# cvsp-lab/ICLR2025_3D-MOM

Hardware: AMD Instinct MI355X
Metric: 4DGS train-steps/sec @200k Gaussians, 960×540, 60 frames; render FPS (higher is better)
Workload: dtype f32; 1 GPU; 200k Gaussians, 60 frames, 960x540, HexPlane on; gaussians=200000, frames=60, width=960, height=540, parallelism=single, ranks_seen=1, gaussians_at_end=200000, steps_replayed_after_overflow=0

## Files before the change

### iclr2025_3d-mom_amd/_native.py

```python
from __future__ import annotations

import ctypes as C
import os
import subprocess

_HERE = os.path.dirname(os.path.abspath(__file__))
LIB_PATH = os.environ.get("MOM4D_LIB") or os.path.join(_HERE, "lib", "libmom4d.so")
_lib = None

MOM_OK, MOM_EINVAL, MOM_ELAUNCH, MOM_ECAPACITY, MOM_EUNAVAILABLE = 0, -1, -2, -3, -4
_ERR = {MOM_EINVAL: "invalid argument", MOM_ELAUNCH: "HIP launch/runtime failure", MOM_ECAPACITY: "scratch too small",
        MOM_EUNAVAILABLE: "run-time dependency missing (librccl)"}
COMM_F32, COMM_I32, COMM_SUM, COMM_MAX = 0, 1, 0, 1


class MomError(RuntimeError):
    pass


GACC_FLOATS = int(os.environ.get("MOM_GACC_FLOATS", "12"))
ABI_VERSION = 8


class MomRasterArgs(C.Structure):
    _fields_ = [("struct_size", C.c_uint),
                ("P", C.c_int), ("D", C.c_int), ("M", C.c_int), ("W", C.c_int), ("H", C.c_int),
                ("background", C.c_void_p), ("means3D", C.c_void_p), ("shs", C.c_void_p), ("shs_rest", C.c_void_p),
                ("colors_precomp", C.c_void_p), ("opacities", C.c_void_p), ("scales", C.c_void_p),
                ("rotations", C.c_void_p), ("cov3D_precomp", C.c_void_p), ("viewmatrix", C.c_void_p),
                ("projmatrix", C.c_void_p), ("campos", C.c_void_p), ("scale_modifier", C.c_float),
                ("tan_fovx", C.c_float), ("tan_fovy", C.c_float), ("prefiltered", C.c_int), ("debug", C.c_int),
                ("tile_row0", C.c_int), ("tile_row1", C.c_int),
                ("forward_only", C.c_int),
                ("overflow_tag", C.c_uint),
                ("keep_all_tiles", C.c_int),
                ("l1_target", C.c_void_p), ("l1_grad", C.c_void_p), ("l1_sums", C.c_void_p),
                ("accum_cleared", C.c_int),
                ("l1_partials", C.c_void_p),
                ("status_post", C.c_void_p), ("status_serial", C.c_uint),
                ("l1_grad_scale", C.c_float),
                ("params_raw", C.c_int)]

    def __init__(self, *args, **kw):
        super().__init__(*args, **kw)
        self.struct_size = C.sizeof(type(self))


class MomRasterGrads(C.Structure):
    _fields_ = [(n, C.c_void_p) for n in ("dL_dmeans2D", "dL_dcolors", "dL_dopacity", "dL_dmeans3D", "dL_dcov3D",
                                          "dL_dsh", "dL_dsh_rest", "dL_dscales", "dL_drotations", "act_rotations_raw",
                                          "dL_dscales_copy", "dL_drotations_copy",
                                          "stats_max_radii2D", "stats_grad_accum", "stats_denom", "stats_skip_if_nonzero")]


class MomRasterAccum(C.Structure):
    _fields_ = [("struct_size", C.c_uint),
                ("dL_dmeans3D_copy", C.c_void_p),
                ("radii_max", C.c_void_p)]

    def __init__(self, *args, **kw):
# ... 283 lines not shown
```

### iclr2025_3d-mom_amd/csrc/raster_api.hip

```cpp
#include "mom_common.h"

int mom_launch_preprocess_fwd(const MomRasterArgs* a, const GeomView& g, int* radii, uint32_t* zero_words, int n_zero, hipStream_t s);
int mom_launch_mark_visible(int P, const float* means3D, const float* view, uint8_t* present, hipStream_t s);
int mom_launch_binning_count(const MomRasterArgs* a, const GeomView& g, const ImageView& im, uint32_t* num_rendered_dev,
                             uint32_t* num_rendered_host, hipStream_t s);
int mom_launch_binning_sort(const MomRasterArgs* a, const GeomView& g, const BinView& b, const ImageView& im, size_t capacity,
                            uint32_t* status_dev, bool render_sorts_small, hipStream_t s);
int mom_launch_render_fwd(const MomRasterArgs* a, const GeomView& g, const BinView& b, const ImageView& im, size_t capacity,
                          float* out_color, float* out_depth, bool sort_small, hipStream_t s);
int mom_launch_render_bwd(const MomRasterArgs* a, const GeomView& g, const BinView& b, const ImageView& im, size_t capacity,
                          const float* dL_dpix, const float* dL_ddepth, hipStream_t s);
int mom_launch_preprocess_bwd(const MomRasterArgs* a, const int* radii, const GeomView& g, const MomRasterGrads* gr, const MomRasterAccum* acc,
                              hipStream_t s);

static int check_args(const MomRasterArgs* a)
{
    if (!a || a->struct_size != sizeof(MomRasterArgs)) return MOM_EINVAL;
    if (a->P < 0 || a->W <= 0 || a->H <= 0) return MOM_EINVAL;
    if (a->tile_row0 < 0 || a->tile_row1 < a->tile_row0 || a->tile_row1 > (a->H + MOM_TILE - 1) / MOM_TILE) return MOM_EINVAL;
    if (a->params_raw && (a->cov3D_precomp || !a->scales || !a->rotations)) return MOM_EINVAL;
    if (a->P == 0) return MOM_OK;
    if (!a->means3D || !a->opacities || !a->viewmatrix || !a->projmatrix || !a->campos || !a->background) return MOM_EINVAL;
    if (!a->shs && !a->colors_precomp) return MOM_EINVAL;
    if (!a->cov3D_precomp && (!a->scales || !a->rotations)) return MOM_EINVAL;
    if (a->shs && !a->colors_precomp && (a->D < 0 || a->D > 3 || a->M < (a->D + 1) * (a->D + 1))) return MOM_EINVAL;
    return MOM_OK;
// ... 70 lines not shown
    out->bin_keys = (size_t)((char*)b.keys - z);
    out->bin_point_list = (size_t)((char*)b.point_list - z);
    out->img_tile_counts = (size_t)((char*)im.tile_counts - z);
    out->img_tile_walked = (size_t)((char*)im.tile_cursor - z);
    return MOM_OK;
}

int mom_raster_forward_geometry(const MomRasterArgs* a, void* geom, void* image, int* radii,
                                uint32_t* num_rendered_dev, uint32_t* num_rendered_host, mom_stream_t stream)
{
    int rc = check_args(a);
    if (rc) return rc;
    hipStream_t s = (hipStream_t)stream;
    if (!num_rendered_dev) return MOM_EINVAL;
    if (a->P == 0) {
        if (hipMemsetAsync(num_rendered_dev, 0, 4, s) != hipSuccess) return MOM_ELAUNCH;
        if (num_rendered_host) *num_rendered_host = 0;
        return MOM_OK;
    }
    if (!geom || !image || !radii) return MOM_EINVAL;
    GeomView g; ImageView im;
    geom_view(mom_align_ptr(geom), a->P, &g);
    image_view(mom_align_ptr(image), a->W, a->H, &im);
    const int tiles = ((a->W + MOM_TILE - 1) / MOM_TILE) * ((a->H + MOM_TILE - 1) / MOM_TILE);
    rc = mom_launch_preprocess_fwd(a, g, radii, im.hdr, (int)((im.tile_counts + tiles) - im.hdr), s);
    if (rc) return rc;
    MOM_CHECK_LAUNCH(a, s);
    rc = mom_launch_binning_count(a, g, im, num_rendered_dev, num_rendered_host, s);
    if (rc) return rc;
    MOM_CHECK_LAUNCH(a, s);
    return MOM_OK;
}

int mom_raster_forward_render(const MomRasterArgs* a, void* geom, void* binning, size_t capacity, void* image,
                              float* out_color, float* out_depth, uint32_t* status_dev, mom_stream_t stream)
{
    int rc = check_args(a);
    if (rc) return rc;
    hipStream_t s = (hipStream_t)stream;
    if (!out_color || !out_depth) return MOM_EINVAL;
    const size_t HW = (size_t)a->W * a->H;
    if (a->P == 0) {
        if (hipMemsetAsync(out_color, 0, HW * 12, s) != hipSuccess) return MOM_ELAUNCH;
        if (hipMemsetAsync(out_depth, 0, HW * 4, s) != hipSuccess) return MOM_ELAUNCH;
        return MOM_OK;
    }
    if (!geom || !binning || !image) return MOM_EINVAL;
    GeomView g; ImageView im; BinView b;
// ... 111 lines not shown
```

### iclr2025_3d-mom_amd/csrc/raster_bin_dev.h

```cpp
#pragma once
#include "mom_common.h"

namespace {

#ifndef MOM_SMALL_RECT
#define MOM_SMALL_RECT 24
#endif
constexpr int kSmallRect = MOM_SMALL_RECT;
constexpr int kMaxLdsTiles = 16384;


struct Reach {
    float cx, cy, a, b, c, bound, inv_a, inv_c;
    int cull;
};
__device__ __forceinline__ bool tile_reached(const Reach& r, int tx, int ty)
{
    if (!r.cull) return true;
    const float xa = (float)(tx * MOM_TILE), ya = (float)(ty * MOM_TILE);
    return mom_rect_reach(r.cx, r.cy, r.a, r.b, r.c, r.bound, r.inv_a, r.inv_c, xa, xa + (float)(MOM_TILE - 1), ya,
                          ya + (float)(MOM_TILE - 1));
}
__device__ __forceinline__ float bcast(float v, int src) { return __int_as_float(__builtin_amdgcn_readlane(__float_as_int(v), src)); }

// ... 42 lines not shown
    while (big) {
        const int src = __ffsll((long long)big) - 1;
        big &= big - 1;
        const WaveSplat b = bcast_splat(x0, y0, w, cnt, 0u, 0ull, rc, src);
        const float inv_w = __builtin_amdgcn_rcpf((float)b.w);
        for (int base = 0; base < b.cnt; base += MOM_WAVE) {
            const int i = base + lane;
            bool r = false;
            if (i < b.cnt) {
                const int q = small_div(i, inv_w);
                const int tx = b.x0 + i - q * b.w, ty = b.y0 + q;
                r = tile_reached(b.rc, tx, ty);
                if (r) f(ty * gx + tx);
            }
            if (base == 0) {
                const uint64_t bal = __ballot(r);
                if (lane == src) mask = bal;
            }
        }
    }
    return mask;
}


}

template <bool LOCAL_STAGES, class KeyPtr>
__device__ __forceinline__ void bitonic_sort(KeyPtr k, int n, int nthreads, int tid)
{
    int lm = 0;
    while ((1 << lm) < n) lm++;
    if (lm == 0) return;
    if (lm == 1) {
        __syncthreads();
        if (tid == 0) { const uint64_t ka = k[0], kb = k[1]; if (ka > kb) { k[0] = kb; k[1] = ka; } }
        __syncthreads();
        return;
    }
    const int quarter_m = (1 << lm) >> 2;
    constexpr uint64_t kInf = ~0ull;
    bool prev_wide = true;
    auto sync_before = [&](int span) {
        const bool wide = !LOCAL_STAGES || span > 256;
        if (wide || prev_wide) __syncthreads();
        else __builtin_amdgcn_wave_barrier();
        prev_wide = wide;
// ... 34 lines not shown
                cx(k0, k1); cx(k2, k3);
                st4(i0, i1, i2, i3, k0, k1, k2, k3);
            }
        }
        int lj = lk - 3;
        for (; lj >= 1; lj -= 2) {
            const int j = 1 << lj, h = j >> 1;
            sync_before(2 * j);
            for (int g = tid; g < quarter_m; g += nthreads) {
                const int x = ((g >> (lj - 1)) << (lj + 1)) | (g & (h - 1));
                const int i0 = x, i1 = x + h, i2 = x + j, i3 = x + j + h;
                if (i1 < n) {
                    uint64_t k0 = k[i0], k1 = k[i1], k2 = ld(i2), k3 = ld(i3);
                    cx(k0, k2); cx(k1, k3);
                    cx(k0, k1); cx(k2, k3);
                    st4(i0, i1, i2, i3, k0, k1, k2, k3);
                }
            }
        }
        if (lj == 0) pairs_pass();
    }
    __syncthreads();
}


constexpr int kRenderSortCap = 1536;
```

### iclr2025_3d-mom_amd/csrc/raster_binning.hip

```cpp
#include "raster_bin_dev.h"

namespace {

constexpr int kSortLdsCap = 8192;
#ifndef MOM_SORT_SMALL
#define MOM_SORT_SMALL 2048
#endif
constexpr int kSortSmallCap = MOM_SORT_SMALL;
constexpr int kOrderBins = 128;

template <class F>
__device__ __forceinline__ void for_each_kept(int x0, int y0, int x1, int y1, int gx, uint32_t payload, uint64_t mask, const Reach& rc, F f)
{
    const int lane = mom_lane();
    const int w = x1 - x0;
    const int cnt = w * (y1 - y0);
    const bool own = cnt <= MOM_WAVE && __popcll(mask) <= kSmallRect;
    if (own && cnt > 0) {
        const float inv_w = __builtin_amdgcn_rcpf((float)w);
        uint64_t m = mask;
        while (m) {
            const int i = __ffsll((long long)m) - 1;
            m &= m - 1;
            const int q = small_div(i, inv_w);
            f((y0 + q) * gx + x0 + i - q * w, lane, payload);
        }
    }
    unsigned long long big = __ballot(!own && cnt > 0);
    while (big) {
        const int src = __ffsll((long long)big) - 1;
        big &= big - 1;
        const WaveSplat b = bcast_splat(x0, y0, w, cnt, payload, mask, rc, src);
        const float inv_w = __builtin_amdgcn_rcpf((float)b.w);
        for (int base = 0; base < b.cnt; base += MOM_WAVE) {
            const int i = base + lane;
            if (i < b.cnt) {
                const int q = small_div(i, inv_w);
                const int tx = b.x0 + i - q * b.w, ty = b.y0 + q;
                const bool r = base == 0 ? ((b.mask >> lane) & 1) : tile_reached(b.rc, tx, ty);
                if (r) f(ty * gx + tx, src, b.payload);
            }
        }
    }
}

struct RectIn {
    float4 r0, r1;
    int radius;
};
__device__ __forceinline__ RectIn fetch_rect(const float4* __restrict__ rec, int g, int P)
{
    RectIn in;
    in.r0 = in.r1 = make_float4(0.f, 0.f, 0.f, 0.f);
    in.radius = 0;
    if (g < P) {
        in.r0 = rec[3 * (size_t)g];
        in.r1 = rec[3 * (size_t)g + 1];
        in.radius = __float_as_int(rec[3 * (size_t)g + 2].w);
    }
    return in;
}
__device__ __forceinline__ void make_rect(const RectIn& in, int gx, int gy, int ry0, int ry1, int cull,
                                          int& x0, int& y0, int& x1, int& y1, uint32_t& depth_bits, Reach& rc)
{
    x0 = y0 = x1 = y1 = 0;
    depth_bits = 0;
    rc = Reach{0.f, 0.f, 0.f, 0.f, 0.f, 0.f, 0.f, 0.f, 0};
    const float4 r0 = in.r0, r1 = in.r1;
    const int radius = in.radius;
    asm volatile("" :: "v"(r0.x), "v"(r0.y), "v"(r0.z), "v"(r1.x), "v"(r1.y), "v"(r1.z), "v"(r1.w), "v"(radius));
    if (radius > 0) {
        mom_get_rect(r0.x, r0.y, radius, gx, gy, x0, y0, x1, y1);
        y0 = max(y0, ry0);
        y1 = min(y1, ry1);
        if (y1 <= y0) x0 = y0 = x1 = y1 = 0;
        depth_bits = __float_as_uint(r0.z);
        if (cull && r1.x > 0.f && r1.z > 0.f)
            rc = Reach{r0.x, r0.y, r1.x, r1.y, r1.z, mom_power_bound(r1.w), __builtin_amdgcn_rcpf(r1.x), __builtin_amdgcn_rcpf(r1.z), 1};
    }
}

template <bool LDS_HIST>
__global__ void __launch_bounds__(256) tile_hist_kernel(int P, int chunks, int gx, int gy, int ry0, int ry1, int cull, const float4* __restrict__ rec,
                                                       uint32_t* __restrict__ tile_counts, unsigned long long* __restrict__ reach)
{
    extern __shared__ uint32_t s_cnt[];
    const int tiles = gx * gy;
    if (LDS_HIST) {
        for (int t = threadIdx.x; t < tiles; t += 256) s_cnt[t] = 0;
        __syncthreads();
    }
    for (int c = 0; c < chunks; c++) {
        const int g = (blockIdx.x * chunks + c) * 256 + threadIdx.x;
        int x0, y0, x1, y1;
        uint32_t db;
        Reach rc;
        make_rect(fetch_rect(rec, g, P), gx, gy, ry0, ry1, cull, x0, y0, x1, y1, db, rc);
        const uint64_t mask = decide_instances(x0, y0, x1, y1, gx, rc, [&](int tile) {
            if (LDS_HIST)
                atomicAdd(&s_cnt[tile], 1u);
            else
                atomicAdd(&tile_counts[tile], 1u);
        });
        if (g < P) reach[g] = mask;
    }
    if (LDS_HIST) {
        __syncthreads();
        for (int t = threadIdx.x; t < tiles; t += 256) {
            const uint32_t n = s_cnt[t];
            if (n) atomicAdd(&tile_counts[t], n);
        }
    }
}

__global__ void __launch_bounds__(1024) tile_scan_kernel(int tiles, const uint32_t* __restrict__ tile_counts,
                                                        uint32_t* __restrict__ tile_cursor, uint2* __restrict__ ranges,
                                                        uint32_t* __restrict__ hdr, uint32_t* __restrict__ num_rendered_dev,
                                                        uint32_t* __restrict__ num_rendered_host, int t0, int nt,
                                                        uint32_t* __restrict__ tile_order)
{
    __shared__ uint32_t s_wave[16];
    __shared__ uint32_t s_carry;
    __shared__ uint32_t s_bin[kOrderBins + 1];
    __shared__ uint32_t s_big;
    const int lane = threadIdx.x & 63, wave = threadIdx.x >> 6;
    if (threadIdx.x == 0) s_carry = 0;
    for (int i = threadIdx.x; i <= kOrderBins; i += 1024) s_bin[i] = 0;
    auto bin_of = [&](uint32_t n) { return kOrderBins - 1 - (int)min((uint32_t)(kOrderBins - 1), n >> 5); };
    __syncthreads();
    for (int base = 0; base < tiles; base += 1024) {
        const int t = base + threadIdx.x;
        const uint32_t n = t < tiles ? tile_counts[t] : 0u;
        if (t >= t0 && t < t0 + nt) atomicAdd(&s_bin[bin_of(n) + 1], 1u);
        uint32_t incl = n;
#pragma unroll
        for (int d = 1; d < 64; d <<= 1) {
            const uint32_t o = __shfl_up(incl, d);
            if (lane >= d) incl += o;
        }
        if (lane == 63) s_wave[wave] = incl;
        __syncthreads();
        uint32_t woff = 0;
        for (int w = 0; w < wave; w++) woff += s_wave[w];
        const uint32_t carry = s_carry;
        const uint32_t start = carry + woff + incl - n;
        if (t < tiles) {
            tile_cursor[t] = start;
            ranges[t] = n ? make_uint2(start, start + n) : make_uint2(0u, 0u);
        }
        __syncthreads();
        if (threadIdx.x == 1023) s_carry = start + n;
        __syncthreads();
    }
    if (threadIdx.x < 64) {
        static_assert(kOrderBins == 128, "two classes per lane of one wave");
        const uint32_t c0 = s_bin[2 * lane + 1], c1 = s_bin[2 * lane + 2];
        uint32_t incl = c0 + c1;
#pragma unroll
        for (int d = 1; d < 64; d <<= 1) {
            const uint32_t o = __shfl_up(incl, d);
            if (lane >= d) incl += o;
        }
        const uint32_t excl = incl - (c0 + c1);
        s_bin[2 * lane] = excl;
        s_bin[2 * lane + 1] = excl + c0;
        static_assert(kRenderSortCap % 32 == 0 && kRenderSortCap / 32 < kOrderBins, "class boundary");
        constexpr int kFirstSmall = kOrderBins - kRenderSortCap / 32;
        if (2 * lane == kFirstSmall) s_big = excl;
        if (2 * lane + 1 == kFirstSmall) s_big = excl + c0;
    }
    __syncthreads();
    for (int t = t0 + threadIdx.x; t < t0 + nt; t += 1024) tile_order[atomicAdd(&s_bin[bin_of(tile_counts[t])], 1u)] = (uint32_t)t;
    if (threadIdx.x == 0) {
        hdr[0] = s_carry;
        hdr[3] = (uint32_t)t0;
        hdr[4] = (uint32_t)nt;
        hdr[5] = s_big;
        *num_rendered_dev = s_carry;
        if (num_rendered_host) __hip_atomic_store(num_rendered_host, s_carry, __ATOMIC_RELAXED, __HIP_MEMORY_SCOPE_SYSTEM);
    }
}

template <bool LDS_HIST>
__global__ void __launch_bounds__(256) tile_scatter_kernel(int P, int chunks, int gx, int gy, int ry0, int ry1, int cull, const float4* __restrict__ rec,
                                                          const unsigned long long* __restrict__ reach,
                                                          uint32_t* __restrict__ tile_cursor, uint64_t* __restrict__ keys,
                                                          uint32_t capacity, uint32_t* __restrict__ hdr, uint32_t* __restrict__ sticky,
                                                          uint32_t tag)
{
    extern __shared__ uint32_t s_cnt[];
    const int tiles = gx * gy;
    bool overflow = false;
    const int g_first = blockIdx.x * chunks * 256 + threadIdx.x;
    RectIn in = fetch_rect(rec, g_first, P);
    unsigned long long rmask = g_first < P ? reach[g_first] : 0ull;
    int x0 = 0, y0 = 0, x1 = 0, y1 = 0;
    uint32_t db = 0;
    Reach rc;
    if (LDS_HIST) {
        for (int t = threadIdx.x; t < tiles; t += 256) s_cnt[t] = 0;
        __syncthreads();
        for (int c = 0; c < chunks; c++) {
            const int g = (blockIdx.x * chunks + c) * 256 + threadIdx.x;
            if (c) {
                rmask = g < P ? reach[g] : 0ull;
                in = fetch_rect(rec, g, P);
            }
            make_rect(in, gx, gy, ry0, ry1, cull, x0, y0, x1, y1, db, rc);
            for_each_kept(x0, y0, x1, y1, gx, 0u, rmask, rc, [&](int tile, int, uint32_t) { atomicAdd(&s_cnt[tile], 1u); });
        }
        __syncthreads();
        for (int t0 = threadIdx.x; t0 < tiles; t0 += 8 * 256) {
            uint32_t n[8], base[8];
#pragma unroll
            for (int k = 0; k < 8; k++) n[k] = t0 + 256 * k < tiles ? s_cnt[t0 + 256 * k] : 0u;
#pragma unroll
            for (int k = 0; k < 8; k++) base[k] = n[k] ? atomicAdd(&tile_cursor[t0 + 256 * k], n[k]) : 0u;
#pragma unroll
            for (int k = 0; k < 8; k++)
                if (n[k]) s_cnt[t0 + 256 * k] = base[k];
        }
        __syncthreads();
    }
    for (int c = 0; c < chunks; c++) {
        const int g = (blockIdx.x * chunks + c) * 256 + threadIdx.x;
        const int wave_g0 = g - mom_lane();
        if (chunks > 1 || !LDS_HIST) {
            rmask = g < P ? reach[g] : 0ull;
            if (c || LDS_HIST) in = fetch_rect(rec, g, P);
            make_rect(in, gx, gy, ry0, ry1, cull, x0, y0, x1, y1, db, rc);
        }
        for_each_kept(x0, y0, x1, y1, gx, db, rmask, rc, [&](int tile, int src, uint32_t sdb) {
            const uint32_t pos = LDS_HIST ? atomicAdd(&s_cnt[tile], 1u) : atomicAdd(&tile_cursor[tile], 1u);
            if (pos < capacity)
                keys[pos] = ((uint64_t)sdb << 32) | (uint32_t)(wave_g0 + src);
            else
                overflow = true;
        });
    }
    if (overflow) {
        atomicOr(&hdr[1], 1u);
        if (sticky) atomicCAS(sticky, 0u, tag);
    }
}

template <int LO, int CAP>
__global__ void __launch_bounds__(256) tile_sort_kernel(const uint2* __restrict__ ranges, const uint32_t* __restrict__ tile_order,
                                                       uint64_t* __restrict__ keys, uint32_t* __restrict__ point_list, uint32_t capacity,
                                                       const uint32_t* __restrict__ head_count, int nt)
{
    __shared__ uint64_t s_keys[CAP];
    const int limit = head_count ? min((int)*head_count, nt) : nt;
    for (int slot = blockIdx.x; slot < limit; slot += gridDim.x) {
        const uint2 r = ranges[tile_order[slot]];
        uint32_t end = r.y < capacity ? r.y : capacity;
        if (r.x >= end) continue;
        const int n = (int)(end - r.x);
        if (n <= LO || (n > CAP && CAP < kSortLdsCap)) continue;
        uint64_t* gk = keys + r.x;
        __syncthreads();
        if (n <= CAP) {
            for (int i = threadIdx.x; i < n; i += 256) s_keys[i] = gk[i];
            __syncthreads();
            if (n > 1) bitonic_sort<true>(s_keys, n, 256, threadIdx.x);
            for (int i = threadIdx.x; i < n; i += 256) point_list[r.x + i] = (uint32_t)s_keys[i];
        } else {
            __syncthreads();
            bitonic_sort<false>(gk, n, 256, threadIdx.x);
            __threadfence_block();
            for (int i = threadIdx.x; i < n; i += 256) point_list[r.x + i] = (uint32_t)gk[i];
        }
    }
}

}

static int bin_chunks(int P)
{
    const int chunks = (P + 256 * 2048 - 1) / (256 * 2048);
    return chunks < 1 ? 1 : chunks;
}

int mom_launch_binning_count(const MomRasterArgs* a, const GeomView& g, const ImageView& im, uint32_t* num_rendered_dev,
                             uint32_t* num_rendered_host, hipStream_t s)
{
    const int gx = (a->W + MOM_TILE - 1) / MOM_TILE, gy = (a->H + MOM_TILE - 1) / MOM_TILE;
    const int tiles = gx * gy;
    int ry0, ry1;
    mom_tile_rows(a, gy, &ry0, &ry1);
    const int cull = a->keep_all_tiles ? 0 : 1;
    const int chunks = bin_chunks(a->P);
    const int blocks = (a->P + 256 * chunks - 1) / (256 * chunks);
    mom_prof_begin(MOM_P_HIST, s);
    if (tiles <= kMaxLdsTiles)
        hipLaunchKernelGGL(tile_hist_kernel<true>, dim3(blocks), dim3(256), (size_t)tiles * 4, s, a->P, chunks, gx, gy, ry0, ry1, cull,
                           g.rec, im.tile_counts, g.reach);
    else
        hipLaunchKernelGGL(tile_hist_kernel<false>, dim3(blocks), dim3(256), 0, s, a->P, chunks, gx, gy, ry0, ry1, cull, g.rec,
                           im.tile_counts, g.reach);
    mom_prof_end(MOM_P_HIST, s);
    if (hipGetLastError() != hipSuccess) return MOM_ELAUNCH;
    MomProfScope ps(MOM_P_SCAN, s);
    hipLaunchKernelGGL(tile_scan_kernel, dim3(1), dim3(1024), 0, s, tiles, im.tile_counts, im.tile_cursor, im.ranges, im.hdr,
                       num_rendered_dev, num_rendered_host, gx * ry0, gx * (ry1 - ry0), im.tile_order);
    return hipGetLastError() == hipSuccess ? MOM_OK : MOM_ELAUNCH;
}

int mom_launch_binning_sort(const MomRasterArgs* a, const GeomView& g, const BinView& b, const ImageView& im, size_t capacity,
                            uint32_t* status_dev, bool render_sorts_small, hipStream_t s)
{
    const int gx = (a->W + MOM_TILE - 1) / MOM_TILE, gy = (a->H + MOM_TILE - 1) / MOM_TILE;
    const int tiles = gx * gy;
    int ry0, ry1;
    mom_tile_rows(a, gy, &ry0, &ry1);
    const int cull = a->keep_all_tiles ? 0 : 1;
    const int chunks = bin_chunks(a->P);
    const int blocks = (a->P + 256 * chunks - 1) / (256 * chunks);
    const uint32_t cap = capacity > 0xFFFFFFFFull ? 0xFFFFFFFFu : (uint32_t)capacity;
    const uint32_t tag = a->overflow_tag ? a->overflow_tag : 1u;
    mom_prof_begin(MOM_P_SCATTER, s);
    if (tiles <= kMaxLdsTiles)
        hipLaunchKernelGGL(tile_scatter_kernel<true>, dim3(blocks), dim3(256), (size_t)tiles * 4, s, a->P, chunks, gx, gy,
                           ry0, ry1, cull, g.rec, g.reach, im.tile_cursor, b.keys, cap, im.hdr, status_dev, tag);
    else
        hipLaunchKernelGGL(tile_scatter_kernel<false>, dim3(blocks), dim3(256), 0, s, a->P, chunks, gx, gy, ry0, ry1, cull, g.rec,
                           g.reach, im.tile_cursor, b.keys, cap, im.hdr, status_dev, tag);
    mom_prof_end(MOM_P_SCATTER, s);
    if (hipGetLastError() != hipSuccess) return MOM_ELAUNCH;
    MomProfScope ps(MOM_P_SORT, s);
    const int nt = gx * (ry1 - ry0);
    if (nt == 0) return MOM_OK;
    if (render_sorts_small) {
        hipLaunchKernelGGL((tile_sort_kernel<kRenderSortCap, kSortLdsCap>), dim3(nt < 128 ? nt : 128), dim3(256), 0, s, im.ranges,
                           im.tile_order, b.keys, b.point_list, cap, im.hdr + 5, nt);
        return hipGetLastError() == hipSuccess ? MOM_OK : MOM_ELAUNCH;
    }
    hipLaunchKernelGGL((tile_sort_kernel<0, kSortSmallCap>), dim3(nt), dim3(256), 0, s, im.ranges, im.tile_order, b.keys, b.point_list,
                       cap, (const uint32_t*)nullptr, nt);
    if (hipGetLastError() != hipSuccess) return MOM_ELAUNCH;
    hipLaunchKernelGGL((tile_sort_kernel<kSortSmallCap, kSortLdsCap>), dim3(nt), dim3(256), 0, s, im.ranges, im.tile_order, b.keys,
                       b.point_list, cap, (const uint32_t*)nullptr, nt);
    return hipGetLastError() == hipSuccess ? MOM_OK : MOM_ELAUNCH;
}
```

### iclr2025_3d-mom_amd/fused_render.py

```python
import ctypes as C
from collections import deque

import torch

from . import _native as N
from . import ops
from .diff_gaussian_rasterization import _C as RC


class FusedRender:
    def __init__(self, gaussians):
        self.g = gaussians
        self.lib = N.lib()
        self.key = None
        self.cap = 0
        self.binning = None
        self._desc_key = None
        self.serial = 0
        self.pending = deque()
        self.collect = False
        self.bad = []

    def _ensure(self, P, W, H, dev):
        if self.key == (P, W, H, dev):
# ... 93 lines not shown

    def _raster(self, a, P, W, H, dev, s):
        lib = self.lib
        a.forward_only = 1
        color = torch.empty((3, H, W), dtype=torch.float32, device=dev)
        depth = torch.empty((1, H, W), dtype=torch.float32, device=dev)
        radii = torch.empty(P, dtype=torch.int32, device=dev)
        prev_R = int(self.nr_host[0])
        late = self.overflowed(self.FLAG_LAG) if len(self.pending) > self.FLAG_LAG else []
        if late and self.collect:
            self.bad += late
        elif late:
            raise N.MomError(f"async render(): frames {late} overflowed the binning capacity and are incomplete; render them "
                             "again (the capacity has been raised), collect such frames with FusedRender.overflowed(), or use "
                             "set_sync_mode('exact')")
        wait_for_count = RC._state["mode"] == "exact" or self.cap == 0
        if wait_for_count:
            if getattr(self, "_unwaited", False):
                torch.cuda.current_stream(dev).synchronize()
                self._unwaited = False
            self.nr_host[0] = RC.COUNT_PENDING
        else:
            self._unwaited = True
        N.check(lib.mom_raster_forward_geometry(C.byref(a), self.geom.data_ptr(), self.img.data_ptr(), radii.data_ptr(),
                                                self.nr_dev.data_ptr(), self.nr_host.data_ptr(), s), "raster_geometry")
        if wait_for_count:
            count = RC.wait_count(self.nr_host)
            want = count + (0 if RC._state["mode"] == "exact" else count // 2 + 65536)
        else:
            want = max(self.cap, int(prev_R * self.HEADROOM) + self.MARGIN, getattr(self, "cap_floor", 0))
        if self.binning is None or want > self.cap or want < self.cap // 4:
            self.cap = want
            self.binning = torch.empty(lib.mom_raster_binning_bytes(P, W, H, self.cap), dtype=torch.uint8, device=dev)
        self.serial += 1
        post = RC._state["mode"] != "exact"
        if post:
            slot = self.serial % self.RING
            a.status_post, a.status_serial = self.flag_ring.data_ptr() + 8 * slot, self.serial & 0xFFFFFFFF
        N.check(lib.mom_raster_forward_render(C.byref(a), self.geom.data_ptr(), self.binning.data_ptr(), self.cap,
                                              self.img.data_ptr(), color.data_ptr(), depth.data_ptr(),
                                              None, s), "raster_render")
        if post:
            self.pending.append((self.serial, slot))
        return color, depth, radii


# ... 58 lines not shown
```

### iclr2025_3d-mom_amd/fused_step.py

```python
import ctypes as C
import os

import torch

from . import _native as N
from . import ops


class _Step:

    RING = 64
    keep_all_tiles = False
    HEADROOM, MARGIN = 1.5, 65536

    def __init__(self, gaussians, opt, hyper, background):
        self.g, self.opt, self.hyper, self.bg = gaussians, opt, hyper, background
        self.P = -1
        self.lib = N.lib()
        self.last = {}
        self.dist = None
        self.next_tag = 1
        self.cap = 0
        self._resize_next = False
        self._bb = None
# ... 72 lines not shown

    def _batch_buffers(self, P, dev):
        b = self._bb
        if b is None or b[0] != (P, dev):
            b = self._bb = ((P, dev), torch.zeros(P, dtype=torch.int32, device=dev), torch.empty(P, 3, dtype=torch.float32, device=dev))
        return b[1], b[2]

    def exact_next(self):
        self._resize_next = True

    def post_flag(self, slot):
        self.flag_ring[slot:slot + 1].copy_(self.flags, non_blocking=True)
        ev = torch.cuda.Event()
        ev.record()
        return ev

    def gather_moments(self):
        """Before an iteration that reads or restructures the optimizer state (FusedStep: sharded Adam).  Here the state is whole."""

    def _raster_forward(self, a, P, W, H, dev, s, radii=None, first=True):
        lib = self.lib
        radii = self.radii if radii is None else radii
        prev_R = int(self.nr_host[0])
        N.check(lib.mom_raster_forward_geometry(C.byref(a), self.geom.data_ptr(), self.img.data_ptr(), radii.data_ptr(),
                                                self.nr_dev.data_ptr(), self.nr_host.data_ptr(), s), "raster_geometry")
        if self.cap == 0 or self._exact_step:
            torch.cuda.current_stream().synchronize()
            prev_R = int(self.nr_host[0])
        want = max(prev_R, int(prev_R * self.HEADROOM) + self.MARGIN)
        if self.binning is None or want > self._bin_cap or (first and want < self._bin_cap // 4):
            self._bin_cap = want
            self.binning = torch.empty(lib.mom_raster_binning_bytes(P, W, H, want), dtype=torch.uint8, device=dev)
        self.cap = self._bin_cap
        N.check(lib.mom_raster_forward_render(C.byref(a), self.geom.data_ptr(), self.binning.data_ptr(), self.cap,
                                              self.img.data_ptr(), self.color.data_ptr(), self.depth.data_ptr(),
                                              self.flags.data_ptr(), s), "raster_render")

    def _ssim_win(self):
        if self.ssim_dm is None:
            (W, H), dev = self._wh, self.color.device
            self.ssim_dm = torch.empty((3, 3, H, W), dtype=torch.float32, device=dev)
            self._ssim_store = torch.empty(1, N.SSIM_SUM_SLOTS, dtype=torch.float64, device=dev)
            self.ssim_sum = self._ssim_store[0]
        return ops._ssim_window()

    def _ssim_full(self, gt, lam, s, k=0, B=1):
        win, (W, H), n = self._ssim_win(), self._wh, self.color.numel()
        sums = self.ssim_sum if B == 1 else self._ssim_sums(B)[k]
        N.check(self.lib.mom_ssim_forward(3, H, W, win, self.color.data_ptr(), gt.data_ptr(), self.ssim_dm.data_ptr(),
# ... 603 lines not shown
```

### iclr2025_3d-mom_amd/ops.py

```python
from __future__ import annotations

import ctypes as C
import math
import os as _os

import numpy as np
import torch

from . import _native as N


def _need_cuda(t, what):
    if not t.is_cuda:
        raise N.MomError(f"{what}: libmom4d has no CPU path (got a {t.device} tensor)")


def plane_storage(p):
    if p.dim() == 4 and p.shape[0] == 1:
        v = p[0].permute(1, 2, 0)
        if v.is_contiguous():
            return v
    return None


# ... 147 lines not shown


def field16_forward(hp, md, P, xyz, time, order, scal, rot, flow, coef, pts, sc_d, rot_d, feat, a0, opac, sc, rot_act, op, s,
                    scratch=None):
    lib = N.lib()
    q = lambda t: None if t is None else t.data_ptr()
    if not lib.mom_deform_field16_supported(C.byref(hp)):
        raise N.MomError(f"field16_forward: {hp.levels} levels of {hp.channels} channels (needs 2 of 16, resolutions <= 1024)")
    N.check(lib.mom_deform_field16_forward(C.byref(hp), C.byref(md), P, xyz.data_ptr(), float(time), q(order), scal.data_ptr(),
                                           rot.data_ptr(), flow.data_ptr(), float(coef), pts.data_ptr(), sc_d.data_ptr(),
                                           rot_d.data_ptr(), q(feat), q(a0), q(opac), q(sc), q(rot_act), q(op), q(scratch), s),
            "deform_field16_fwd")


def gaussian_params(g, who):
    ps = g._xyz.data, g._features_dc.data, g._features_rest.data, g._scaling.data, g._rotation.data, g._opacity.data
    for t in ps:
        if not t.is_contiguous():
            raise N.MomError(f"{who}: the Gaussian parameters must be contiguous")
    return ps


def raster_args(cam, view, proj, campos, bg, P, D, means, f_dc, f_rest, opac, scales, rots, params_raw, scale_modifier, debug,
                keep_all_tiles):
    a = N.MomRasterArgs()
    a.P, a.D, a.M, a.W, a.H = P, D, 16, int(cam.image_width), int(cam.image_height)
    a.background, a.means3D = bg.data_ptr(), means.data_ptr()
    a.shs, a.shs_rest = f_dc.data_ptr(), f_rest.data_ptr()
    a.opacities, a.scales, a.rotations = opac.data_ptr(), scales.data_ptr(), rots.data_ptr()
    a.params_raw = int(params_raw)
    a.viewmatrix, a.projmatrix, a.campos = view.data_ptr(), proj.data_ptr(), campos.data_ptr()
    a.scale_modifier = float(scale_modifier)
    a.tan_fovx, a.tan_fovy = math.tan(cam.FoVx * 0.5), math.tan(cam.FoVy * 0.5)
    a.debug = int(bool(debug))
    a.keep_all_tiles = int(keep_all_tiles)
    return a


def raster_grads(g2d, gcol, gop, gxyz, gcov, gdc, grest, gsc, grot):
    gr = N.MomRasterGrads()
    gr.dL_dmeans2D, gr.dL_dcolors, gr.dL_dopacity = g2d.data_ptr(), gcol.data_ptr(), gop.data_ptr()
    gr.dL_dmeans3D, gr.dL_dcov3D = gxyz.data_ptr(), gcov.data_ptr()
    gr.dL_dsh, gr.dL_dsh_rest = gdc.data_ptr(), grest.data_ptr()
    gr.dL_dscales, gr.dL_drotations = gsc.data_ptr(), grot.data_ptr()
    return gr


class DeformMLPFunction(torch.autograd.Function):

    @staticmethod
    def _desc(params, grads=None):
        d = N.MomDeformMLP()
        W0, b0, *rest = params
        d.W0, d.b0 = W0.data_ptr(), b0.data_ptr()
        for k in range(3):
            W1, b1, W2, b2 = rest[4 * k:4 * k + 4]
            d.W1[k], d.b1[k], d.W2[k], d.b2[k] = W1.data_ptr(), b1.data_ptr(), W2.data_ptr(), b2.data_ptr()
        if grads is not None:
# ... 648 lines not shown
```

### include/mom4d.h

```cpp
#ifndef MOM4D_H_INCLUDED
#define MOM4D_H_INCLUDED

#include <stddef.h>
#include <stdint.h>

#ifdef __cplusplus
extern "C" {
#endif

#define MOM_OK 0
#define MOM_EINVAL (-1)
#define MOM_ELAUNCH (-2)
#define MOM_ECAPACITY (-3)
#define MOM_EUNAVAILABLE (-4)

#define MOM_TILE 16

typedef void* mom_stream_t;

#define MOM_ABI_VERSION 8
#ifndef MOM_GACC_FLOATS
#define MOM_GACC_FLOATS 12
#endif
int mom_abi_version(void);
// ... 13 lines not shown
    const float* means3D;
    const float* shs;
    const float* shs_rest;
    const float* colors_precomp;
    const float* opacities;
    const float* scales;
    const float* rotations;
    const float* cov3D_precomp;
    const float* viewmatrix;
    const float* projmatrix;
    const float* campos;
    float scale_modifier;
    float tan_fovx, tan_fovy;
    int prefiltered;
    int debug;
    int tile_row0, tile_row1;
    int forward_only;
    uint32_t overflow_tag;
    int keep_all_tiles;
    const float* l1_target;
    float* l1_grad;
    float* l1_sums;
    int accum_cleared;
    float* l1_partials;
    unsigned long long* status_post;
    uint32_t status_serial;
    float l1_grad_scale;
    int params_raw;
} MomRasterArgs;

size_t mom_raster_geom_bytes(int P);
size_t mom_raster_image_bytes(int W, int H);
size_t mom_raster_binning_bytes(int P, int W, int H, size_t capacity );

int mom_raster_forward_geometry(const MomRasterArgs* a, void* geom, void* image, int* radii,
                                uint32_t* num_rendered_dev, uint32_t* num_rendered_host, mom_stream_t stream);

int mom_raster_forward_render(const MomRasterArgs* a, void* geom, void* binning, size_t capacity, void* image,
                              float* out_color, float* out_depth, uint32_t* status_dev, mom_stream_t stream);

typedef struct MomRasterGrads {
    float* dL_dmeans2D;
    float* dL_dcolors;
    float* dL_dopacity;
    float* dL_dmeans3D;
    float* dL_dcov3D;
// ... 220 lines not shown
```

Measured before the change: 1175 steps/s.

## Fold tile-count scan into scatter kernel when host does not wait for count

When the caller does not need the rendered count synchronously, the single-block tile_scan kernel is skipped. Each scatter block instead recomputes the prefix scan of tile counts into LDS, and block 0 writes the ranges, tile order and count header. This removes a serial one-block launch between histogram and scatter, at the cost of every scatter block redundantly scanning about 2k tiles and doubling its LDS use. It also adds optional timing stamps behind a compile flag.

```diff
diff --git a/iclr2025_3d-mom_amd/_native.py b/iclr2025_3d-mom_amd/_native.py
--- a/iclr2025_3d-mom_amd/_native.py
+++ b/iclr2025_3d-mom_amd/_native.py
@@ -36,6 +36,7 @@
                 ("keep_all_tiles", C.c_int),
                 ("l1_target", C.c_void_p), ("l1_grad", C.c_void_p), ("l1_sums", C.c_void_p),
                 ("accum_cleared", C.c_int),
+                ("count_in_scatter", C.c_int),
                 ("l1_partials", C.c_void_p),
                 ("status_post", C.c_void_p), ("status_serial", C.c_uint),
                 ("l1_grad_scale", C.c_float),
diff --git a/iclr2025_3d-mom_amd/csrc/raster_api.hip b/iclr2025_3d-mom_amd/csrc/raster_api.hip
--- a/iclr2025_3d-mom_amd/csrc/raster_api.hip
+++ b/iclr2025_3d-mom_amd/csrc/raster_api.hip
@@ -2,6 +2,7 @@
 
 int mom_launch_preprocess_fwd(const MomRasterArgs* a, const GeomView& g, int* radii, uint32_t* zero_words, int n_zero, hipStream_t s);
 int mom_launch_mark_visible(int P, const float* means3D, const float* view, uint8_t* present, hipStream_t s);
+int mom_binning_zero_words(const MomRasterArgs* a, const ImageView& im);
 int mom_launch_binning_count(const MomRasterArgs* a, const GeomView& g, const ImageView& im, uint32_t* num_rendered_dev,
                              uint32_t* num_rendered_host, hipStream_t s);
 int mom_launch_binning_sort(const MomRasterArgs* a, const GeomView& g, const BinView& b, const ImageView& im, size_t capacity,
@@ -118,8 +119,7 @@
     GeomView g; ImageView im;
     geom_view(mom_align_ptr(geom), a->P, &g);
     image_view(mom_align_ptr(image), a->W, a->H, &im);
-    const int tiles = ((a->W + MOM_TILE - 1) / MOM_TILE) * ((a->H + MOM_TILE - 1) / MOM_TILE);
-    rc = mom_launch_preprocess_fwd(a, g, radii, im.hdr, (int)((im.tile_counts + tiles) - im.hdr), s);
+    rc = mom_launch_preprocess_fwd(a, g, radii, im.hdr, mom_binning_zero_words(a, im), s);
     if (rc) return rc;
     MOM_CHECK_LAUNCH(a, s);
     rc = mom_launch_binning_count(a, g, im, num_rendered_dev, num_rendered_host, s);
diff --git a/iclr2025_3d-mom_amd/csrc/raster_bin_dev.h b/iclr2025_3d-mom_amd/csrc/raster_bin_dev.h
--- a/iclr2025_3d-mom_amd/csrc/raster_bin_dev.h
+++ b/iclr2025_3d-mom_amd/csrc/raster_bin_dev.h
@@ -1,5 +1,7 @@
 #pragma once
 #include "mom_common.h"
+
+constexpr int kRenderSortCap = 1536;
 
 namespace {
 
@@ -88,6 +90,98 @@
     return mask;
 }
 
+
+constexpr int kOrderBins = 128;
+__device__ __forceinline__ int order_bin(uint32_t n) { return kOrderBins - 1 - (int)min((uint32_t)(kOrderBins - 1), n >> 5); }
+
+template <int NT, int PER, class Emit>
+__device__ __forceinline__ uint32_t scan_tile_counts(int tiles, const uint32_t* __restrict__ tile_counts, uint32_t* s_wave, Emit emit)
+{
+    constexpr int NW = NT / 64;
+    const int lane = threadIdx.x & 63, wave = threadIdx.x >> 6;
+    uint32_t carry = 0;
+    int half = 0;
+    for (int base = 0; base < tiles; base += NT * PER, half ^= NW) {
+        const int t = base + (int)threadIdx.x * PER;
+        uint32_t n[PER];
+        bool whole = false;
+        if constexpr (PER % 4 == 0) whole = t + PER <= tiles;
+        if (whole) {
+#pragma unroll
+            for (int k = 0; k + 3 < PER; k += 4) {
+                const uint4 v = *reinterpret_cast<const uint4*>(tile_counts + t + k);
+                n[k] = v.x; n[k + 1] = v.y; n[k + 2] = v.z; n[k + 3] = v.w;
+            }
+        } else {
+#pragma unroll
+            for (int k = 0; k < PER; k++) n[k] = t + k < tiles ? tile_counts[t + k] : 0u;
+        }
+        uint32_t sum = 0;
+#pragma unroll
+        for (int k = 0; k < PER; k++) sum += n[k];
+        uint32_t incl = sum;
+#pragma unroll
+        for (int d = 1; d < 64; d <<= 1) {
+            const uint32_t o = __shfl_up(incl, d);
+            if (lane >= d) incl += o;
+        }
+        if (lane == 63) s_wave[half + wave] = incl;
+        __syncthreads();
+        uint32_t woff = 0, all = 0;
+#pragma unroll
+        for (int w = 0; w < NW; w++) {
+            const uint32_t v = s_wave[half + w];
+            if (w < wave) woff += v;
+            all += v;
+        }
+        uint32_t start = carry + woff + incl - sum;
+#pragma unroll
+        for (int k = 0; k < PER; k++) {
+            if (t + k < tiles) emit(t + k, n[k], start);
+            start += n[k];
+        }
+        carry += all;
+    }
+    return carry;
+}
+
+template <int NT, class Count>
+__device__ __forceinline__ uint32_t build_tile_order(int t0, int nt, uint32_t* s_bin, uint32_t* s_big, uint32_t* __restrict__ tile_order,
+                                                     Count count)
+{
+    const int lane = threadIdx.x & 63;
+    if (threadIdx.x < 64) {
+        static_assert(kOrderBins == 128, "two classes per lane of one wave");
+        const uint32_t c0 = s_bin[2 * lane + 1], c1 = s_bin[2 * lane + 2];
+        uint32_t incl = c0 + c1;
+#pragma unroll
+        for (int d = 1; d < 64; d <<= 1) {
+            const uint32_t o = __shfl_up(incl, d);
+            if (lane >= d) incl += o;
+        }
+        const uint32_t excl = incl - (c0 + c1);
+        s_bin[2 * lane] = excl;
+        s_bin[2 * lane + 1] = excl + c0;
+        static_assert(kRenderSortCap % 32 == 0 && kRenderSortCap / 32 < kOrderBins, "class boundary");
+        constexpr int kFirstSmall = kOrderBins - kRenderSortCap / 32;
+        if (2 * lane == kFirstSmall) *s_big = excl;
+        if (2 * lane + 1 == kFirstSmall) *s_big = excl + c0;
+    }
+    __syncthreads();
+    for (int t = t0 + (int)threadIdx.x; t < t0 + nt; t += NT) tile_order[atomicAdd(&s_bin[order_bin(count(t))], 1u)] = (uint32_t)t;
+    return *s_big;
+}
+
+__device__ __forceinline__ void write_count_header(uint32_t* __restrict__ hdr, uint32_t total, int t0, int nt, uint32_t big,
+                                                   uint32_t* num_rendered_dev, uint32_t* num_rendered_host)
+{
+    hdr[0] = total;
+    hdr[3] = (uint32_t)t0;
+    hdr[4] = (uint32_t)nt;
+    hdr[5] = big;
+    if (num_rendered_dev) *num_rendered_dev = total;
+    if (num_rendered_host) __hip_atomic_store(num_rendered_host, total, __ATOMIC_RELAXED, __HIP_MEMORY_SCOPE_SYSTEM);
+}
 
 }
 
@@ -168,6 +262,3 @@
     }
     __syncthreads();
 }
-
-
-constexpr int kRenderSortCap = 1536;
diff --git a/iclr2025_3d-mom_amd/csrc/raster_binning.hip b/iclr2025_3d-mom_amd/csrc/raster_binning.hip
--- a/iclr2025_3d-mom_amd/csrc/raster_binning.hip
+++ b/iclr2025_3d-mom_amd/csrc/raster_binning.hip
@@ -7,7 +7,8 @@
 #define MOM_SORT_SMALL 2048
 #endif
 constexpr int kSortSmallCap = MOM_SORT_SMALL;
-constexpr int kOrderBins = 128;
+constexpr int kMaxFoldTiles = 8192;
+constexpr int kHdrCountPtrs = 8;
 
 template <class F>
 __device__ __forceinline__ void for_each_kept(int x0, int y0, int x1, int y1, int gx, uint32_t payload, uint64_t mask, const Reach& rc, F f)
@@ -44,6 +45,45 @@
     }
 }
 
+#ifdef FWD_STAMPS
+constexpr int kBinStampWords = 8, kBinStampWaves = 16384;
+__device__ unsigned long long g_bin_stamps[2][kBinStampWaves * kBinStampWords];
+struct BinStamp {
+    unsigned long long r0, c0, n_big, tiles_big, passes;
+};
+__device__ __forceinline__ void bin_stamp_begin(BinStamp& b)
+{
+    b.r0 = __builtin_amdgcn_s_memrealtime();
+    b.c0 = __builtin_amdgcn_s_memtime();
+    b.n_big = b.tiles_big = b.passes = 0;
+}
+__device__ __forceinline__ void bin_stamp_work(BinStamp& b, bool big, int cnt)
+{
+    b.n_big += __popcll(__ballot(big));
+    int v = big ? cnt : 0, p = big ? (cnt + MOM_WAVE - 1) / MOM_WAVE : 0;
+    for (int d = 32; d; d >>= 1) {
+        v += __shfl_xor(v, d);
+        p += __shfl_xor(p, d);
+    }
+    b.tiles_big += v;
+    b.passes += p;
+}
+__device__ __forceinline__ void bin_stamp_end(const BinStamp& b, int kernel)
+{
+    asm volatile("s_waitcnt vmcnt(0) lgkmcnt(0)" ::: "memory");
+    const int w = blockIdx.x * 4 + (threadIdx.x >> 6);
+    if ((threadIdx.x & 63) == 0 && w < kBinStampWaves) {
+        unsigned long long* o = g_bin_stamps[kernel] + (size_t)w * kBinStampWords;
+        o[0] = b.r0; o[1] = __builtin_amdgcn_s_memrealtime();
+        o[2] = b.c0; o[3] = __builtin_amdgcn_s_memtime();
+        o[4] = b.n_big; o[5] = b.tiles_big; o[6] = b.passes; o[7] = 1;
+    }
+}
+#define BIN_STAMP(x) x
+#else
+#define BIN_STAMP(x)
+#endif
+
 struct RectIn {
     float4 r0, r1;
     int radius;
@@ -82,10 +122,17 @@
 
 template <bool LDS_HIST>
 __global__ void __launch_bounds__(256) tile_hist_kernel(int P, int chunks, int gx, int gy, int ry0, int ry1, int cull, const float4* __restrict__ rec,
-                                                       uint32_t* __restrict__ tile_counts, unsigned long long* __restrict__ reach)
+                                                       uint32_t* __restrict__ tile_counts, unsigned long long* __restrict__ reach,
+                                                       uint32_t* __restrict__ count_ptrs, uint32_t* num_rendered_dev,
+                                                       uint32_t* num_rendered_host)
 {
     extern __shared__ uint32_t s_cnt[];
     const int tiles = gx * gy;
+    BIN_STAMP(BinStamp bs; bin_stamp_begin(bs);)
+    if (count_ptrs && blockIdx.x == 0 && threadIdx.x == 0) {
+        reinterpret_cast<uint32_t**>(count_ptrs)[0] = num_rendered_dev;
+        reinterpret_cast<uint32_t**>(count_ptrs)[1] = num_rendered_host;
+    }
     if (LDS_HIST) {
         for (int t = threadIdx.x; t < tiles; t += 256) s_cnt[t] = 0;
         __syncthreads();
@@ -96,6 +143,7 @@
         uint32_t db;
         Reach rc;
         make_rect(fetch_rect(rec, g, P), gx, gy, ry0, ry1, cull, x0, y0, x1, y1, db, rc);
+        BIN_STAMP(bin_stamp_work(bs, (x1 - x0) * (y1 - y0) > kSmallRect, (x1 - x0) * (y1 - y0));)
         const uint64_t mask = decide_instances(x0, y0, x1, y1, gx, rc, [&](int tile) {
             if (LDS_HIST)
                 atomicAdd(&s_cnt[tile], 1u);
@@ -111,6 +159,7 @@
             if (n) atomicAdd(&tile_counts[t], n);
         }
     }
+    BIN_STAMP(bin_stamp_end(bs, 0);)
 }
 
 __global__ void __launch_bounds__(1024) tile_scan_kernel(int tiles, const uint32_t* __restrict__ tile_counts,
@@ -119,77 +168,38 @@
                                                         uint32_t* __restrict__ num_rendered_host, int t0, int nt,
                                                         uint32_t* __restrict__ tile_order)
 {
-    __shared__ uint32_t s_wave[16];
-    __shared__ uint32_t s_carry;
+    __shared__ uint32_t s_wave[2 * 16];
     __shared__ uint32_t s_bin[kOrderBins + 1];
     __shared__ uint32_t s_big;
-    const int lane = threadIdx.x & 63, wave = threadIdx.x >> 6;
-    if (threadIdx.x == 0) s_carry = 0;
     for (int i = threadIdx.x; i <= kOrderBins; i += 1024) s_bin[i] = 0;
-    auto bin_of = [&](uint32_t n) { return kOrderBins - 1 - (int)min((uint32_t)(kOrderBins - 1), n >> 5); };
+    const uint32_t total = scan_tile_counts<1024, 1>(tiles, tile_counts, s_wave, [&](int t, uint32_t n, uint32_t start) {
+        if (t >= t0 && t < t0 + nt) atomicAdd(&s_bin[order_bin(n) + 1], 1u);
+        tile_cursor[t] = start;
+        ranges[t] = n ? make_uint2(start, start + n) : make_uint2(0u, 0u);
+    });
     __syncthreads();
-    for (int base = 0; base < tiles; base += 1024) {
-        const int t = base + threadIdx.x;
-        const uint32_t n = t < tiles ? tile_counts[t] : 0u;
-        if (t >= t0 && t < t0 + nt) atomicAdd(&s_bin[bin_of(n) + 1], 1u);
-        uint32_t incl = n;
-#pragma unroll
-        for (int d = 1; d < 64; d <<= 1) {
-            const uint32_t o = __shfl_up(incl, d);
-            if (lane >= d) incl += o;
-        }
-        if (lane == 63) s_wave[wave] = incl;
-        __syncthreads();
-        uint32_t woff = 0;
-        for (int w = 0; w < wave; w++) woff += s_wave[w];
-        const uint32_t carry = s_carry;
-        const uint32_t start = carry + woff + incl - n;
-        if (t < tiles) {
-            tile_cursor[t] = start;
-            ranges[t] = n ? make_uint2(start, start + n) : make_uint2(0u, 0u);
-        }
-        __syncthreads();
-        if (threadIdx.x == 1023) s_carry = start + n;
-        __syncthreads();
-    }
-    if (threadIdx.x < 64) {
-        static_assert(kOrderBins == 128, "two classes per lane of one wave");
-        const uint32_t c0 = s_bin[2 * lane + 1], c1 = s_bin[2 * lane + 2];
-        uint32_t incl = c0 + c1;
-#pragma unroll
-        for (int d = 1; d < 64; d <<= 1) {
-            const uint32_t o = __shfl_up(incl, d);
-            if (lane >= d) incl += o;
-        }
-        const uint32_t excl = incl - (c0 + c1);
-        s_bin[2 * lane] = excl;
-        s_bin[2 * lane + 1] = excl + c0;
-        static_assert(kRenderSortCap % 32 == 0 && kRenderSortCap / 32 < kOrderBins, "class boundary");
-        constexpr int kFirstSmall = kOrderBins - kRenderSortCap / 32;
-        if (2 * lane == kFirstSmall) s_big = excl;
-        if (2 * lane + 1 == kFirstSmall) s_big = excl + c0;
-    }
-    __syncthreads();
-    for (int t = t0 + threadIdx.x; t < t0 + nt; t += 1024) tile_order[atomicAdd(&s_bin[bin_of(tile_counts[t])], 1u)] = (uint32_t)t;
-    if (threadIdx.x == 0) {
-        hdr[0] = s_carry;
-        hdr[3] = (uint32_t)t0;
-        hdr[4] = (uint32_t)nt;
-        hdr[5] = s_big;
-        *num_rendered_dev = s_carry;
-        if (num_rendered_host) __hip_atomic_store(num_rendered_host, s_carry, __ATOMIC_RELAXED, __HIP_MEMORY_SCOPE_SYSTEM);
-    }
-}
-
-template <bool LDS_HIST>
+    const uint32_t big = build_tile_order<1024>(t0, nt, s_bin, &s_big, tile_order, [&](int t) { return tile_counts[t]; });
+    if (threadIdx.x == 0) write_count_header(hdr, total, t0, nt, big, num_rendered_dev, num_rendered_host);
+}
+
+struct FoldArgs {
+    const uint32_t* tile_counts;
+    uint2* ranges;
+    uint32_t* tile_order;
+    int t0, nt;
+};
+template <bool LDS_HIST, bool FOLD>
 __global__ void __launch_bounds__(256) tile_scatter_kernel(int P, int chunks, int gx, int gy, int ry0, int ry1, int cull, const float4* __restrict__ rec,
                                                           const unsigned long long* __restrict__ reach,
                                                           uint32_t* __restrict__ tile_cursor, uint64_t* __restrict__ keys,
                                                           uint32_t capacity, uint32_t* __restrict__ hdr, uint32_t* __restrict__ sticky,
-                                                          uint32_t tag)
-{
+                                                          uint32_t tag, FoldArgs fa)
+{
+    static_assert(LDS_HIST || !FOLD, "the folded scan keeps the bucket starts beside the LDS histogram");
     extern __shared__ uint32_t s_cnt[];
     const int tiles = gx * gy;
+    uint32_t* s_start = s_cnt + tiles;
+    BIN_STAMP(BinStamp bs; bin_stamp_begin(bs);)
     bool overflow = false;
     const int g_first = blockIdx.x * chunks * 256 + threadIdx.x;
     RectIn in = fetch_rect(rec, g_first, P);
@@ -199,7 +209,33 @@
     Reach rc;
     if (LDS_HIST) {
         for (int t = threadIdx.x; t < tiles; t += 256) s_cnt[t] = 0;
-        __syncthreads();
+        if constexpr (FOLD) {
+            __shared__ uint32_t s_wave[2 * 4];
+            __shared__ uint32_t s_bin[kOrderBins + 1];
+            __shared__ uint32_t s_big;
+            const bool writer = blockIdx.x == 0;
+            if (writer)
+                for (int i = threadIdx.x; i <= kOrderBins; i += 256) s_bin[i] = 0;
+            const uint32_t total = scan_tile_counts<256, 8>(tiles, fa.tile_counts, s_wave, [&](int t, uint32_t n, uint32_t start) {
+                s_start[t] = start;
+                if (writer) {
+                    if (t >= fa.t0 && t < fa.t0 + fa.nt) atomicAdd(&s_bin[order_bin(n) + 1], 1u);
+                    fa.ranges[t] = n ? make_uint2(start, start + n) : make_uint2(0u, 0u);
+                }
+            });
+            if (writer) {
+                __syncthreads();
+                const uint32_t big = build_tile_order<256>(fa.t0, fa.nt, s_bin, &s_big, fa.tile_order, [&](int t) {
+                    return (t + 1 < tiles ? s_start[t + 1] : total) - s_start[t];
+                });
+                if (threadIdx.x == 0) {
+                    uint32_t* const* ptrs = reinterpret_cast<uint32_t* const*>(hdr + kHdrCountPtrs);
+                    write_count_header(hdr, total, fa.t0, fa.nt, big, ptrs[0], ptrs[1]);
+                }
+            }
+        } else {
+            __syncthreads();
+        }
         for (int c = 0; c < chunks; c++) {
             const int g = (blockIdx.x * chunks + c) * 256 + threadIdx.x;
             if (c) {
@@ -218,7 +254,7 @@
             for (int k = 0; k < 8; k++) base[k] = n[k] ? atomicAdd(&tile_cursor[t0 + 256 * k], n[k]) : 0u;
 #pragma unroll
             for (int k = 0; k < 8; k++)
-                if (n[k]) s_cnt[t0 + 256 * k] = base[k];
+                if (n[k]) s_cnt[t0 + 256 * k] = base[k] + (FOLD ? s_start[t0 + 256 * k] : 0u);
         }
         __syncthreads();
     }
@@ -230,6 +266,7 @@
             if (c || LDS_HIST) in = fetch_rect(rec, g, P);
             make_rect(in, gx, gy, ry0, ry1, cull, x0, y0, x1, y1, db, rc);
         }
+        BIN_STAMP(bin_stamp_work(bs, (x1 - x0) * (y1 - y0) > 0 && !((x1 - x0) * (y1 - y0) <= MOM_WAVE && __popcll(rmask) <= kSmallRect), (x1 - x0) * (y1 - y0));)
         for_each_kept(x0, y0, x1, y1, gx, db, rmask, rc, [&](int tile, int src, uint32_t sdb) {
             const uint32_t pos = LDS_HIST ? atomicAdd(&s_cnt[tile], 1u) : atomicAdd(&tile_cursor[tile], 1u);
             if (pos < capacity)
@@ -242,6 +279,7 @@
         atomicOr(&hdr[1], 1u);
         if (sticky) atomicCAS(sticky, 0u, tag);
     }
+    BIN_STAMP(bin_stamp_end(bs, 1);)
 }
 
 template <int LO, int CAP>
@@ -281,6 +319,13 @@
     return chunks < 1 ? 1 : chunks;
 }
 
+static bool fold_scan(const MomRasterArgs* a, int tiles) { return a->count_in_scatter != 0 && tiles <= kMaxFoldTiles; }
+int mom_binning_zero_words(const MomRasterArgs* a, const ImageView& im)
+{
+    const int tiles = ((a->W + MOM_TILE - 1) / MOM_TILE) * ((a->H + MOM_TILE - 1) / MOM_TILE);
+    return (int)(((fold_scan(a, tiles) ? im.tile_cursor : im.tile_counts) + tiles) - im.hdr);
+}
+
 int mom_launch_binning_count(const MomRasterArgs* a, const GeomView& g, const ImageView& im, uint32_t* num_rendered_dev,
                              uint32_t* num_rendered_host, hipStream_t s)
 {
@@ -291,15 +336,18 @@
     const int cull = a->keep_all_tiles ? 0 : 1;
     const int chunks = bin_chunks(a->P);
     const int blocks = (a->P + 256 * chunks - 1) / (256 * chunks);
+    const bool fold = fold_scan(a, tiles);
+    uint32_t* count_ptrs = fold ? im.hdr + kHdrCountPtrs : nullptr;
     mom_prof_begin(MOM_P_HIST, s);
     if (tiles <= kMaxLdsTiles)
         hipLaunchKernelGGL(tile_hist_kernel<true>, dim3(blocks), dim3(256), (size_t)tiles * 4, s, a->P, chunks, gx, gy, ry0, ry1, cull,
-                           g.rec, im.tile_counts, g.reach);
+                           g.rec, im.tile_counts, g.reach, count_ptrs, num_rendered_dev, num_rendered_host);
     else
         hipLaunchKernelGGL(tile_hist_kernel<false>, dim3(blocks), dim3(256), 0, s, a->P, chunks, gx, gy, ry0, ry1, cull, g.rec,
-                           im.tile_counts, g.reach);
+                           im.tile_counts, g.reach, count_ptrs, num_rendered_dev, num_rendered_host);
     mom_prof_end(MOM_P_HIST, s);
     if (hipGetLastError() != hipSuccess) return MOM_ELAUNCH;
+    if (fold) return MOM_OK;
     MomProfScope ps(MOM_P_SCAN, s);
     hipLaunchKernelGGL(tile_scan_kernel, dim3(1), dim3(1024), 0, s, tiles, im.tile_counts, im.tile_cursor, im.ranges, im.hdr,
                        num_rendered_dev, num_rendered_host, gx * ry0, gx * (ry1 - ry0), im.tile_order);
@@ -318,13 +366,17 @@
     const int blocks = (a->P + 256 * chunks - 1) / (256 * chunks);
     const uint32_t cap = capacity > 0xFFFFFFFFull ? 0xFFFFFFFFu : (uint32_t)capacity;
     const uint32_t tag = a->overflow_tag ? a->overflow_tag : 1u;
+    const FoldArgs fa = {im.tile_counts, im.ranges, im.tile_order, gx * ry0, gx * (ry1 - ry0)};
     mom_prof_begin(MOM_P_SCATTER, s);
-    if (tiles <= kMaxLdsTiles)
-        hipLaunchKernelGGL(tile_scatter_kernel<true>, dim3(blocks), dim3(256), (size_t)tiles * 4, s, a->P, chunks, gx, gy,
-                           ry0, ry1, cull, g.rec, g.reach, im.tile_cursor, b.keys, cap, im.hdr, status_dev, tag);
+    if (fold_scan(a, tiles))
+        hipLaunchKernelGGL((tile_scatter_kernel<true, true>), dim3(blocks), dim3(256), (size_t)tiles * 8, s, a->P, chunks, gx, gy,
+                           ry0, ry1, cull, g.rec, g.reach, im.tile_cursor, b.keys, cap, im.hdr, status_dev, tag, fa);
+    else if (tiles <= kMaxLdsTiles)
+        hipLaunchKernelGGL((tile_scatter_kernel<true, false>), dim3(blocks), dim3(256), (size_t)tiles * 4, s, a->P, chunks, gx, gy,
+                           ry0, ry1, cull, g.rec, g.reach, im.tile_cursor, b.keys, cap, im.hdr, status_dev, tag, fa);
     else
-        hipLaunchKernelGGL(tile_scatter_kernel<false>, dim3(blocks), dim3(256), 0, s, a->P, chunks, gx, gy, ry0, ry1, cull, g.rec,
-                           g.reach, im.tile_cursor, b.keys, cap, im.hdr, status_dev, tag);
+        hipLaunchKernelGGL((tile_scatter_kernel<false, false>), dim3(blocks), dim3(256), 0, s, a->P, chunks, gx, gy, ry0, ry1, cull, g.rec,
+                           g.reach, im.tile_cursor, b.keys, cap, im.hdr, status_dev, tag, fa);
     mom_prof_end(MOM_P_SCATTER, s);
     if (hipGetLastError() != hipSuccess) return MOM_ELAUNCH;
     MomProfScope ps(MOM_P_SORT, s);
@@ -342,3 +394,13 @@
                        b.point_list, cap, (const uint32_t*)nullptr, nt);
     return hipGetLastError() == hipSuccess ? MOM_OK : MOM_ELAUNCH;
 }
+
+#ifdef FWD_STAMPS
+extern "C" int mom_debug_bin_stamps(unsigned long long* host_dst, int kernel, int waves)
+{
+    if (kernel < 0 || kernel > 1) return MOM_EINVAL;
+    if (waves > kBinStampWaves) waves = kBinStampWaves;
+    return hipMemcpyFromSymbol(host_dst, HIP_SYMBOL(g_bin_stamps), (size_t)waves * kBinStampWords * 8,
+                               (size_t)kernel * kBinStampWaves * kBinStampWords * 8) == hipSuccess ? MOM_OK : MOM_ELAUNCH;
+}
+#endif
diff --git a/iclr2025_3d-mom_amd/fused_render.py b/iclr2025_3d-mom_amd/fused_render.py
--- a/iclr2025_3d-mom_amd/fused_render.py
+++ b/iclr2025_3d-mom_amd/fused_render.py
@@ -139,6 +139,7 @@
             self.nr_host[0] = RC.COUNT_PENDING
         else:
             self._unwaited = True
+        a.count_in_scatter = 0 if wait_for_count else 1
         N.check(lib.mom_raster_forward_geometry(C.byref(a), self.geom.data_ptr(), self.img.data_ptr(), radii.data_ptr(),
                                                 self.nr_dev.data_ptr(), self.nr_host.data_ptr(), s), "raster_geometry")
         if wait_for_count:
diff --git a/iclr2025_3d-mom_amd/fused_step.py b/iclr2025_3d-mom_amd/fused_step.py
--- a/iclr2025_3d-mom_amd/fused_step.py
+++ b/iclr2025_3d-mom_amd/fused_step.py
@@ -118,9 +118,11 @@
         lib = self.lib
         radii = self.radii if radii is None else radii
         prev_R = int(self.nr_host[0])
+        wait = self.cap == 0 or self._exact_step
+        a.count_in_scatter = 0 if wait else 1
         N.check(lib.mom_raster_forward_geometry(C.byref(a), self.geom.data_ptr(), self.img.data_ptr(), radii.data_ptr(),
                                                 self.nr_dev.data_ptr(), self.nr_host.data_ptr(), s), "raster_geometry")
-        if self.cap == 0 or self._exact_step:
+        if wait:
             torch.cuda.current_stream().synchronize()
             prev_R = int(self.nr_host[0])
         want = max(prev_R, int(prev_R * self.HEADROOM) + self.MARGIN)
diff --git a/iclr2025_3d-mom_amd/ops.py b/iclr2025_3d-mom_amd/ops.py
--- a/iclr2025_3d-mom_amd/ops.py
+++ b/iclr2025_3d-mom_amd/ops.py
@@ -193,7 +193,7 @@
 
 
 def raster_args(cam, view, proj, campos, bg, P, D, means, f_dc, f_rest, opac, scales, rots, params_raw, scale_modifier, debug,
-                keep_all_tiles):
+                keep_all_tiles, count_in_scatter=0):
     a = N.MomRasterArgs()
     a.P, a.D, a.M, a.W, a.H = P, D, 16, int(cam.image_width), int(cam.image_height)
     a.background, a.means3D = bg.data_ptr(), means.data_ptr()
@@ -205,6 +205,7 @@
     a.tan_fovx, a.tan_fovy = math.tan(cam.FoVx * 0.5), math.tan(cam.FoVy * 0.5)
     a.debug = int(bool(debug))
     a.keep_all_tiles = int(keep_all_tiles)
+    a.count_in_scatter = int(count_in_scatter)
     return a
 
 
diff --git a/include/mom4d.h b/include/mom4d.h
--- a/include/mom4d.h
+++ b/include/mom4d.h
@@ -59,6 +59,7 @@
     float* l1_grad;
     float* l1_sums;
     int accum_cleared;
+    int count_in_scatter;
     float* l1_partials;
     unsigned long long* status_post;
     uint32_t status_serial;
```

New measurement: 1181 steps/s (median of 3 runs). No clear change (+0.6%).
